# PlantandFoodResearch/MCHap

Hardware: AMD Instinct MI355X
Metric: loci/sec (whole node) for 1000-step MCMC, tetraploid 8-SNV loci, 1/2/4/8 GPUs (higher is better)
Workload: dtype f64; 1 GPU; 10000 synthetic tetraploid loci per GPU, 8 SNVs, 200 reads, 1000 MCMC steps x 2 chains, burn 500, posterior summary (BASELINE.json configs[1]); 4 passes in flight on separate HIP streams, each with its own device buffers; loci_per_gpu=10000, ploidy=4, snvs=8, reads=200, mcmc_steps=1000, chains=2, burn=500, llk_cache=True, passes_in_flight=4, hw_queues=4, world_size=1, devices=1

## Files before the change

mchap_amd/csrc/denovo_spec_kernel.hpp:

```cpp
#pragma once
#include <type_traits>

#include "denovo_simt_kernel.hpp"

#ifdef MCHAP_MASK_PADDING
#define MCHAP_PAD_LANE(x) (x)
#else
#define MCHAP_PAD_LANE(x) true
#endif
#ifndef MCHAP_COOP_UNR
#define MCHAP_COOP_UNR 2
#endif
#ifndef MCHAP_SPEC_TB
#define MCHAP_SPEC_TB 4
#endif
#ifndef MCHAP_SPEC_LOW
#define MCHAP_SPEC_LOW 8
#endif
#ifndef MCHAP_SPEC_CG
#define MCHAP_SPEC_CG 4
#endif
#ifndef MCHAP_SPEC_VAR
#define MCHAP_SPEC_VAR 0
#endif
// ... 42 lines not shown
  static __device__ __forceinline__ CT ld(u8 p) { return *reinterpret_cast<GLBP(const CT)>(p); }
};
template <>
struct TabPtr<true> {
  typedef LDSP(const uint8_t) u8;
  typedef LDSP(const double) f64;
  template <class CT>
  static __device__ __forceinline__ CT ld(u8 p) { return *reinterpret_cast<LDSP(const CT)>(p); }
};

enum { GP_RT = 0, GP_CW, GP_CT, GP_CACHE, GP_CKEYS, GP_TRACE, GP_LLK, GP_GBP, GP_N };
enum { GV_INB = 0, GV_MLO, GV_MHI, GV_N };
struct SpecLds {
  LDSP(uint64_t) pw;
  LDSP(uint64_t) wst;
  LDSP(double) llk_t;
  LDSP(uint64_t) rngn;
  LDSP(double) prior;
  LDSP(double) ptab;
  LDSP(double) optp;
  LDSP(double) optl;
  LDSP(double) ln;
  LDSP(double) lninv;
  LDSP(uint32_t) ivse;
  LDSP(uint32_t) ivlin;
  LDSP(uint32_t) ivlout;
  LDSP(uint32_t) ivno;
  LDSP(uint16_t) cols;
  LDSP(uint16_t) permtab;
  LDSP(uint8_t) shift;
  LDSP(uint8_t) nal;
  LDSP(uint8_t) ktab;
  LDSP(uint8_t) ordtab;
  LDSP(uint16_t) nreads;
  LDSP(uint16_t) ndict;
  LDSP(double) dict;
  LDSP(uint64_t) gptr;
  LDSP(double) gval;
  LDSP(uint32_t) gstream;
  LDSP(uint64_t) bw;
  LDSP(double) bpc;
  LDSP(uint64_t) bpt;
  LDSP(uint64_t) gbt;
  LDSP(const uint8_t) sct;
  LDSP(uint64_t) tbuf;
  LDSP(uint64_t) lc;
  uint32_t lc_mask;
  uint32_t cache_mask;
  int key_words;
  bool cache_on;
  uint64_t epoch = 0ull;
  bool reuse_on;
  bool cut_off = false;
  LDSP(const uint8_t) lds_ct;
  LDSP(const double) lds_cw;
  int crow;
  LDSP(uint64_t) draws;
  LDSP(double) memo_tot;
  LDSP(double) bdist;
  int memo_stride;
  int ndraws;
  LDSP(unsigned char) cx_lds;
  LDSP(double) cx_val;
  uint64_t *cx_base = nullptr;
  int cx_n = 0;
};

__host__ __device__ inline int spec_memo_entries(int Mmax) { return Mmax * (Mmax + 1) / 2; }
__host__ __device__ inline int spec_memo_index(int start, int stop) { return stop * (stop - 1) / 2 + start; }
__host__ __device__ inline size_t spec_memo_bytes(int Mmax, int T, int G) {
  const size_t per_group = (size_t)2 * spec_memo_entries(Mmax) * 8;
  if (T != 1 || per_group > 16 * 1024) return 0;
  return per_group * (64 / G);
}

constexpr int SPEC_LC_ENTRIES = 256;
#ifndef MCHAP_LC_GEN
#define MCHAP_LC_GEN 48
#endif
constexpr uint32_t SPEC_LC_SECOND_LEVEL_GEN = MCHAP_LC_GEN;
__host__ __device__ inline size_t spec_lc_bytes(int entries = SPEC_LC_ENTRIES) { return (size_t)16 * entries + 16; }
__host__ __device__ inline bool spec_ctx_in_bpc(int K, int Mmax, int Amax, int max_reads) {
  return K >= 3 && max_reads <= 64 && Mmax * Amax <= 24 * (K - 2) && 16 * K * Mmax <= 3 * 64 * 8 && 12 * 64 + 4 * 8 <= 3 * 64 * 8;
}
__host__ __device__ inline int spec_lc_entries(int bp_cache) { return (bp_cache & 2) ? ((bp_cache & 4) ? SPEC_LC_ENTRIES / 2 : SPEC_LC_ENTRIES) : 0; }
__device__ __forceinline__ uint32_t sct_off(uint32_t row) { return (row / 24u) * (uint32_t)(4 * WAVE * 8) + (row % 24u) * (uint32_t)WAVE; }
__host__ __device__ inline size_t spec_bp_cache_bytes(int K) { return (size_t)8 * K * 4 * 64 + (size_t)8 * (K + 1); }

constexpr int COAST_NW_LIST = 4;
__host__ __device__ inline size_t coast_lds_bytes(int Mmax) {
  return (size_t)8 * (2 * spec_memo_entries(Mmax) + Mmax) + (size_t)8 * 12;
}

__host__ __device__ inline size_t spec_lds_bytes(int K, int Mmax, int Amax, int T, int G) {
  const int NG = 64 / G;
  const int nmax = K * Mmax;
  const int nopt = Amax > 1 ? Amax - 1 : 1;
  const int niv = Mmax + 1;
  size_t b = 0;
  b += (size_t)8 * K * 64;
  b += (size_t)8 * NG * T * K;
  b += (size_t)8 * NG * T * 2;
  b += (size_t)8 * NG * (2 * K + 5);
  b += (size_t)8 * 64;
  b += (size_t)8 * nopt * 64 * 2;
  b += (size_t)8 * SPEC_LN * 2;
// ... 611 lines not shown
#pragma unroll
  for (int i = 0; i < RPL; i++) acc[i] = 0.0;
#pragma unroll
  for (int h = 0; h < KT; h++) {
    const uint64_t a = S.pw[(size_t)h * WAVE + src], b = S.bw[(size_t)sg * KT + h];
    const bool same = __builtin_amdgcn_readfirstlane((int)(a == b)) != 0;
    double ph[RPL];
    if (same) {
#pragma unroll
      for (int i = 0; i < RPL; i++) ph[i] = bpv[h][i];
    } else {
      spec_hap_prod<RPL, CT, LT>(dict, rows, h * Mh, Mh, ct, crow, ph);
    }
#pragma unroll
    for (int i = 0; i < RPL; i++) acc[i] += ph[i] * invK;
  }
  double wv[RPL];
#pragma unroll
  for (int i = 0; i < RPL; i++) wv[i] = cw[WAVE * i];
  return read_log_sum<RPL>(acc, wv, grouped);
}
template <int KT, int RPL, class CT, bool LT = false, class BP>
__device__ __forceinline__ void spec_base_products(const SpecLds &S, int sg, int mmax, int Mh, uint32_t amask,
                                                   typename TabPtr<LT>::u8 ct, int crow, int lane, BP &bp) {
  LDSP(double) dict = S.dict + (size_t)sg * DICT_MAX;
  const PairRows rows = spec_pair_rows<KT>(S.bw + (size_t)sg * KT, 1, 0, S, sg, mmax, Mh, amask, lane);
#pragma unroll
  for (int h = 0; h < KT; h++) {
    double ph[RPL];
    spec_hap_prod<RPL, CT, LT>(dict, rows, h * Mh, Mh, ct, crow, ph);
#pragma unroll
    for (int i = 0; i < RPL; i++) bp.set(h, i, lane, ph[i]);
  }
}
template <int KT, int RPL, class CT, bool LT = false, class BP>
__device__ __forceinline__ void spec_base_products_of(const SpecLds &S, const PairRows rows, int sg, int h, int Mh,
                                                      typename TabPtr<LT>::u8 ct, int crow, int lane, BP &bp) {
  LDSP(double) dict = S.dict + (size_t)sg * DICT_MAX;
  double ph[RPL];
  spec_hap_prod<RPL, CT, LT>(dict, rows, h * Mh, Mh, ct, crow, ph);
#pragma unroll
  for (int i = 0; i < RPL; i++) bp.set(h, i, lane, ph[i]);
}

template <int KT>
__device__ __forceinline__ unsigned long long spec_same_request(LDSP(uint64_t) pwbuf, unsigned long long reqs, int src, int lane) {
  if ((reqs & (reqs - 1ull)) == 0ull) return reqs;
  bool eq = ((reqs >> lane) & 1ull) != 0ull;
#pragma unroll
  for (int h = 0; h < KT; h++) eq = eq & (pwbuf[(size_t)h * WAVE + lane] == pwbuf[(size_t)h * WAVE + src]);
  return __ballot(eq);
}

template <int KT, int G, bool LT = false, bool DEDUP = true>
__device__ __forceinline__ double spec_coop_all(unsigned long long todo, LDSP(uint64_t) pwbuf, LDSP(uint8_t) shift_tab,
                                                LDSP(uint16_t) cols_tab, LDSP(uint16_t) nreads_tab, LDSP(uint16_t) ndict_tab,
                                                LDSP(double) dict_tab, LDSP(uint64_t) gptr_tab, LDSP(uint64_t) bw_tab,
                                                bool reuse, int crow, int mmax, int Mh_lane, uint32_t amask_lane, int rpad,
                                                int lane, LDSP(const uint8_t) lds_ct = nullptr, LDSP(const double) lds_cw = nullptr,
                                                LDSP(double) bpc = nullptr, LDSP(uint64_t) bpt = nullptr,
                                                LDSP(const uint8_t) sct = nullptr, LDSP(uint64_t) gbt = nullptr) {
  SpecLds S;
  S.pw = pwbuf;
  S.shift = shift_tab;
  S.cols = cols_tab;
  S.dict = dict_tab;
  S.bw = bw_tab;
  const int nch_batch = rpad / WAVE;
  double val = 0.0;
  while (todo) {
    const int sg = (__ffsll((long long)todo) - 1) / G;
    const unsigned long long gmask = G == 64 ? ~0ull : (((1ull << (G & 63)) - 1ull) << (sg * (G & 63)));
    unsigned long long reqs = todo & gmask;
    todo &= ~gmask;
    const int first = __ffsll((long long)reqs) - 1;
    const int Mh = __builtin_amdgcn_readfirstlane(__shfl(Mh_lane, first, WAVE));
    const uint32_t amask = (uint32_t)__builtin_amdgcn_readfirstlane(__shfl((int)amask_lane, first, WAVE));
    LDSP(uint64_t) gp = gptr_tab + sg * GP_N;
    GLBP(const double) rt = (GLBP(const double))(uintptr_t)gp[GP_RT] + lane;
    typename TabPtr<LT>::f64 cw;
    if constexpr (LT) cw = lds_cw + lane;
    else cw = (GLBP(const double))(uintptr_t)gp[GP_CW] + lane;
    const int nrd = (int)nreads_tab[sg];
    const bool grouped = nd_w01(ndict_tab[sg]);
    const int nch = max(1, min(nch_batch, (nrd + WAVE - 1) / WAVE));
    const int cstride = crow / WAVE;
    if (MCHAP_REUSE_MAXK >= KT && nd_count(ndict_tab[sg]) != 0 && KT * Mh <= (MCHAP_SPEC_DEEP ? 3 : 2) * WAVE) {
      const int nb0 = nch < 4 ? nch : 4;
      typename TabPtr<LT>::u8 ct;
      if constexpr (LT) ct = lds_ct + (size_t)lane * cstride;
      else ct = (GLBP(const uint8_t))(uintptr_t)gp[GP_CT] + (size_t)lane * cstride;
      constexpr bool BPL = (G == 64) && !LT;
      bool cached = false;
      if (BPL && bpc != nullptr) {
        bool eq = bpt[KT] != 0ull;
#pragma unroll
        for (int h = 0; h < KT; h++) eq = eq & (bpt[h] == bw_tab[(size_t)sg * KT + h]);
        cached = __builtin_amdgcn_readfirstlane((int)eq) != 0;
      }
      const bool use_base = reuse && (!BPL || bpc != nullptr) && (cached || __popcll(reqs) >= 2);
      BaseProducts<KT, BPL> bp;
      if constexpr (BPL) {
        bp.p = bpc;
      } else {
#pragma unroll
        for (int h = 0; h < KT; h++)
#pragma unroll
          for (int i = 0; i < 4; i++) bp.v[h][i] = 0.0;
      }
      if (use_base && !cached) {
        if constexpr (BPL) {
          const bool any_valid = bpt[KT] != 0ull;
#if MCHAP_SPEC_SBS
          if (sct != nullptr && nch == 1) {
// ... 293 lines not shown
                }
#pragma unroll
                for (int k = 0; k < 4; k++) acc[k] += ph[k] * invK;
              }
#pragma unroll
              for (int k = 0; k < 4; k++)
                if (k < RK) v[k] = read_log(acc[k]) * cwr[k];
            }
            const double a0 = RK > 2 ? v[0] + v[2] : v[0];
            const double a1 = RK > 3 ? v[1] + v[3] : v[1];
            double sv = RK > 1 ? a0 + a1 : a0;
#pragma unroll
            for (int o = 8; o >= 1; o >>= 1) sv += __shfl_xor(sv, o, WAVE);
#pragma unroll
            for (int k = 0; k < 4; k++) {
              const double vk = __shfl(sv, 16 * k, WAVE);
              if (k < nq && ((dupm[k] >> lane) & 1ull)) val = vk;
            }
          }
          continue;
        }
      }
#endif
      while (reqs) {
        const int src = __ffsll((long long)reqs) - 1;
        const unsigned long long dups = (DEDUP ? spec_same_request<KT>(pwbuf, reqs, src, lane) : (1ull << src));
        reqs &= ~dups;
        double s = 0.0;
        if (nb0 == 1) s += spec_coop_reuse<KT, 1, uint8_t, LT>(S, src, sg, mmax, Mh, amask, ct, cw, crow, lane, bp, use_base, grouped);
        else if (nb0 == 2) s += spec_coop_reuse<KT, 2, uint16_t, LT>(S, src, sg, mmax, Mh, amask, ct, cw, crow, lane, bp, use_base, grouped);
        else if (nb0 == 3) s += spec_coop_reuse<KT, 3, uint32_t, LT>(S, src, sg, mmax, Mh, amask, ct, cw, crow, lane, bp, use_base, grouped);
        else s += spec_coop_reuse<KT, 4, uint32_t, LT>(S, src, sg, mmax, Mh, amask, ct, cw, crow, lane, bp, use_base, grouped);
        for (int cb = 4; cb < nch; cb += 4) {
          const int rem = nch - cb;
          typename TabPtr<LT>::f64 cwb = cw + cb * WAVE;
          if (deep) {
            BaseProductsG<KT> bg;
            bg.p = gbp;
            bg.rpad = rpad;
            bg.cb = cb;
            if (rem >= 4) s += spec_coop_reuse_g<KT, 4, uint32_t, LT>(S, src, sg, mmax, Mh, amask, ct + cb, cwb, crow, lane, bg, grouped);
            else if (rem == 3) s += spec_coop_reuse_g<KT, 3, uint32_t, LT>(S, src, sg, mmax, Mh, amask, ct + cb, cwb, crow, lane, bg, grouped);
            else if (rem == 2) s += spec_coop_reuse_g<KT, 2, uint16_t, LT>(S, src, sg, mmax, Mh, amask, ct + cb, cwb, crow, lane, bg, grouped);
            else s += spec_coop_reuse_g<KT, 1, uint8_t, LT>(S, src, sg, mmax, Mh, amask, ct + cb, cwb, crow, lane, bg, grouped);
          } else {
            if (rem >= 4) s += spec_coop_coded<KT, 4, uint32_t, LT>(S, src, sg, mmax, Mh, amask, ct + cb, cwb, crow, lane, grouped);
            else if (rem == 3) s += spec_coop_coded<KT, 3, uint32_t, LT>(S, src, sg, mmax, Mh, amask, ct + cb, cwb, crow, lane, grouped);
            else if (rem == 2) s += spec_coop_coded<KT, 2, uint16_t, LT>(S, src, sg, mmax, Mh, amask, ct + cb, cwb, crow, lane, grouped);
            else s += spec_coop_coded<KT, 1, uint8_t, LT>(S, src, sg, mmax, Mh, amask, ct + cb, cwb, crow, lane, grouped);
          }
        }
        s = wave_sum(s);
        if ((dups >> lane) & 1ull) val = s;
      }
    } else {
      while (reqs) {
        const int src = __ffsll((long long)reqs) - 1;
        const unsigned long long dups = (DEDUP ? spec_same_request<KT>(pwbuf, reqs, src, lane) : (1ull << src));
        reqs &= ~dups;
        double s = 0.0;
        const bool coded = nd_count(ndict_tab[sg]) != 0;
        typename TabPtr<LT>::u8 ct;
        if constexpr (LT) ct = lds_ct + (size_t)lane * cstride;
        else ct = (GLBP(const uint8_t))(uintptr_t)gp[GP_CT] + (size_t)lane * cstride;
        GLBP(const double) cwg = (GLBP(const double))(uintptr_t)gp[GP_CW] + lane;
        for (int cb = 0; cb < nch; cb += 4) {
          const int rem = nch - cb;
          typename TabPtr<LT>::f64 cwb = cw + cb * WAVE;
          if (coded) {
            if (rem >= 4) s += spec_coop_coded<KT, 4, uint32_t, LT>(S, src, sg, mmax, Mh, amask, ct + cb, cwb, crow, lane, grouped);
            else if (rem == 3) s += spec_coop_coded<KT, 3, uint32_t, LT>(S, src, sg, mmax, Mh, amask, ct + cb, cwb, crow, lane, grouped);
            else if (rem == 2) s += spec_coop_coded<KT, 2, uint16_t, LT>(S, src, sg, mmax, Mh, amask, ct + cb, cwb, crow, lane, grouped);
            else s += spec_coop_coded<KT, 1, uint8_t, LT>(S, src, sg, mmax, Mh, amask, ct + cb, cwb, crow, lane, grouped);
          } else {
            GLBP(const double) rtb = rt + cb * WAVE;
            GLBP(const double) cwgb = cwg + cb * WAVE;
            if (rem >= 4) s += spec_coop_body<KT, 4>(S, src, sg, mmax, Mh, amask, rtb, cwgb, rpad, lane, nrd - cb * WAVE, grouped);
            else if (rem == 3) s += spec_coop_body<KT, 3>(S, src, sg, mmax, Mh, amask, rtb, cwgb, rpad, lane, nrd - cb * WAVE, grouped);
            else if (rem == 2) s += spec_coop_body<KT, 2>(S, src, sg, mmax, Mh, amask, rtb, cwgb, rpad, lane, nrd - cb * WAVE, grouped);
            else s += spec_coop_body<KT, 1>(S, src, sg, mmax, Mh, amask, rtb, cwgb, rpad, lane, nrd - cb * WAVE, grouped);
          }
        }
        s = wave_sum(s);
        if ((dups >> lane) & 1ull) val = s;
      }
    }
  }
  return val;
}

struct SpecKeepAll {
  __device__ __forceinline__ bool operator()(bool miss, double) const { return miss; }
};
template <int KT, int G, bool LT = false, class Filter = SpecKeepAll, bool DEDUP = true>
__device__ __forceinline__ double spec_eval(bool need, const GWords<KT> pw, const Grp<KT> &c, const SpecLds &S, int mmax,
                                            int rpad, int lane, Filter filt = Filter()) {
  double val = 0.0;
  if (c.flat) {
    val = c.llk;
    need = false;
  }
  bool miss = need;
  uint64_t tag = 0;
  ulonglong2 *slot = nullptr;
  GSUB_T0();
  const bool wide = C_KEYBITS(c) * KT > 63;
  uint64_t *kslot = nullptr;
  LDSP(uint64_t) lslot = S.lc;
  bool promote = false;
  if (need && S.cache_on) {
    tag = tag_of<KT>(pw, C_KEYBITS(c), S.epoch);
    const uint64_t key = tag >> 1;
    uint32_t hsh = (uint32_t)key ^ ((uint32_t)(key >> 32) * 0x9E3779B1u);
    hsh ^= hsh >> 16;
    hsh *= 0x7FEB352Du;
    hsh ^= hsh >> 15;
    hsh *= 0x846CA68Bu;
    hsh ^= hsh >> 16;
    const size_t set_i = (size_t)((hsh >> 12) & S.cache_mask);
    ulonglong2 *set = reinterpret_cast<ulonglong2 *>((uintptr_t)S.gptr[(lane / G) * GP_N + GP_CACHE]) + 8 * set_i;
    int way = (int)((hsh >> 24) & 7u);
    if (S.lc_mask != 0u && !wide) {
      LDSP(uint64_t) le = S.lc + 2 * (size_t)((hsh >> 3) & S.lc_mask);
      const uint64_t t = le[0], v = le[1];
      if (t == tag) {
        val = __longlong_as_double((long long)v);
        miss = false;
      }
      lslot = le;
      if (miss && c.gen > SPEC_LC_SECOND_LEVEL_GEN) {
#pragma unroll
        for (int w = 7; w >= 0; w--) {
          const ulonglong2 e = set[w];
          if (e.x == tag) {
            val = __longlong_as_double((long long)e.y);
            miss = false;
          }
        }
        promote = !miss;
      }
    } else {
    int hit_way = -1;
#pragma unroll
    for (int w = 7; w >= 0; w--) {
      const ulonglong2 e = set[w];
      if (e.x == tag) {
        val = __longlong_as_double((long long)e.y);
        miss = false;
        hit_way = w;
      }
      if (e.x == 0ull || (S.epoch != 0ull && (e.x ^ S.epoch) >> 33 != 0ull)) way = w;
    }
    if (wide) {
      uint64_t *kset = reinterpret_cast<uint64_t *>((uintptr_t)S.gptr[(lane / G) * GP_N + GP_CKEYS]) + 8 * set_i * S.key_words;
      if (hit_way >= 0) {
        const uint64_t *kw = kset + (size_t)hit_way * S.key_words;
        bool same = true;
#pragma unroll
        for (int h = 0; h < KT; h++) same = same & (kw[h] == pw.w[h]);
        if (!same) {
          miss = true;
          way = hit_way;
        }
      }
      kslot = kset + (size_t)way * S.key_words;
    }
    }
    slot = set + way;
  }
  if (wave_any(promote)) {
    if (promote) lslot[0] = tag;
    lds_sync();
    if (promote && lslot[0] == tag) lslot[1] = (uint64_t)__double_as_longlong(val);
    lds_sync();
  }
  miss = filt(miss, val);
  STAT_ADD(0, need);
  STAT_ADD(1, miss);
  STAT_ADD(2, true);
  unsigned long long todo = __ballot(miss);
  GSUB(c, 9);
  if (todo) {
    GCOUNT(c, 11, __popcll(todo));
    if (miss) {
#pragma unroll
      for (int h = 0; h < KT; h++) S.pw[(size_t)h * WAVE + lane] = pw.w[h];
    }
    if (S.reuse_on && lane % G == 0) {
      const GWords<KT> cg = c.g;
#pragma unroll
      for (int h = 0; h < KT; h++) S.bw[(size_t)(lane / G) * KT + h] = cg.w[h];
    }
    lds_sync();
    const double v = spec_coop_all<KT, G, LT, DEDUP>(todo, S.pw, S.shift, S.cols, S.nreads, S.ndict, S.dict, S.gptr, S.bw, S.reuse_on, S.crow, mmax, c.Mh, C_AMASK(c), rpad, lane, S.lds_ct, S.lds_cw, S.bpc, S.bpt, S.sct, S.gbt);
    if (miss) val = v;
    bool writer = miss && slot != nullptr;
    if (wave_any(writer && wide)) {
      unsigned long long pend = __ballot(writer);
      bool mine = false;
      while (pend) {
        const int l = __ffsll((long long)pend) - 1;
        const unsigned long long sl = __shfl((unsigned long long)(uintptr_t)slot, l, WAVE);
        const unsigned long long same = __ballot(writer && (unsigned long long)(uintptr_t)slot == sl);
        if (lane == l) mine = true;
        pend &= ~same;
      }
      writer = mine;
    }
    if (writer) {
      if (wide) {
#pragma unroll
        for (int h = 0; h < KT; h++) kslot[h] = pw.w[h];
      }
      *slot = make_ulonglong2(tag, (unsigned long long)__double_as_longlong(val));
    }
    if (S.lc_mask != 0u && !wide) {
      if (writer) lslot[0] = tag;
      lds_sync();
      if (writer && lslot[0] == tag) lslot[1] = (uint64_t)__double_as_longlong(val);
    }
    lds_sync();
    GSUB(c, 10);
  }
  return val;
}

#ifndef MCHAP_SPEC_WPE
#define MCHAP_SPEC_WPE 2
#endif

template <int KT, int G, bool LT = false, bool CTX = false>
__device__ __forceinline__ void spec_mutation(Grp<KT> &c, const SpecLds &S, double temp, int amax, int mmax, int nmax, int rpad,
                                              int lane, int gi, int gl) {
  const int Mh = c.Mh;
  const int n = KT * Mh;
  const uint64_t ctr0 = c.ctr;
  bool run = c.alive;
  if (wave_any(c.alive && c.mvalid)) {
    LDSP(uint64_t) utab = S.draws + gi * S.ndraws;
    const bool fast = c.alive && c.mvalid && n <= S.ndraws;
    const int cnt = max(n, min(S.ndraws, 2 * G * ((n / 2 + G) / G) - 1));
    stage_draws<G>(ld_stream(S, gi), ctr0 + (uint64_t)(n - 1), cnt, utab, gl, fast);
    lds_sync();
    bool ok = true;
    if (fast) {
      const double mlo = S.gval[gi * GV_N + GV_MLO], mhi = S.gval[gi * GV_N + GV_MHI];
      for (int p = gl; p < n; p += G) {
        const double u = draw_double(utab[p]);
        ok = ok && (mlo <= u) && (u < mhi);
      }
    }
    const bool bad = grp_ballot<G>(!ok, gi) != 0ull;
    lds_sync();
    if (fast && !bad) {
      c.ctr = ctr0 + (uint64_t)(n - 1) + (uint64_t)n;
      c.doff = n;
      c.dcount = cnt;
      run = false;
    }
  }
  if (run) c.dcount = 0;
  STAT_WAVE(8, 1);
  GPHASE(c, 0);
  if (!wave_any(run)) return;
  STAT_WAVE(9, 1);
// ... 30 lines not shown
  for (int s = 0; s < NS; s++) xs[s] = gl + s * G;
  if constexpr (G == 64) {
    const int nl = __builtin_amdgcn_readfirstlane(run ? n : 0);
    if (nl <= 64) {
      for (int i = nl - 1; i >= 1; i--) {
        const int ki = __builtin_amdgcn_readlane(kv[0], i);
        xs[0] = (xs[0] == i) ? ki : ((xs[0] == ki) ? i : xs[0]);
      }
    } else {
#pragma unroll
      for (int s2 = NS - 1; s2 >= 0; s2--) {
        const int hi = min(nl - 1, s2 * 64 + 63), lo = max(1, s2 * 64);
        for (int i = hi; i >= lo; i--) {
          const int ki = __builtin_amdgcn_readlane(kv[s2], i & 63);
#pragma unroll
          for (int s = 0; s < NS; s++) xs[s] = (xs[s] == i) ? ki : ((xs[s] == ki) ? i : xs[s]);
        }
      }
    }
  } else {
    const int nloop = run ? n : 0;
    int nl = nloop;
#pragma unroll
    for (int o = 32; o >= 1; o >>= 1) nl = max(nl, __shfl_xor(nl, o, WAVE));
    for (int i = nl - 1; i >= 1; i--) {
      if (i < nloop) {
        const int ki = ktab[i];
#pragma unroll
        for (int s = 0; s < NS; s++) xs[s] = (xs[s] == i) ? ki : ((xs[s] == ki) ? i : xs[s]);
      }
    }
  }
  if (run) {
#pragma unroll
    for (int s = 0; s < NS; s++) {
      const int e = gl + s * G;
      if (e < n) {
        int h = 0, j = e;
        while (j >= Mh) {
          j -= Mh;
          h++;
        }
        permtab[xs[s]] = (uint16_t)((h << 8) | j);
      }
    }
  }
  lds_sync();
  if (run) c.ctr = ctr0 + (uint64_t)(n - 1) + (uint64_t)n;
  const int nslots = (NS > 2 && wave_any(c.alive && n > 2 * G)) ? 3 : (two ? 2 : 1);
  const int nrd_ = (int)S.nreads[gi];
  const int wmin = (MCHAP_SPEC_SBS != 0 && G == 64 && S.bpc != nullptr && (nrd_ <= 16 || (nrd_ > 32 && nrd_ <= 64))) ? 4 : MCHAP_SPEC_WIN_MIN;
  bool cx = false;
  if constexpr (CTX && G == 64) cx = S.cx_base != nullptr && amax == 2 && run && c.gen > (uint32_t)MCHAP_CTX_GEN && c.gen >= CXP_ST(S)[CX_PAUSE];
  const bool cut_on = amax == 2 && !S.cut_off && ((S.cache_on && wave_any(c.alive && c.gen > SPEC_LC_SECOND_LEVEL_GEN)) || cx);
  int start = 0;
  int win = max(c.mwin, wmin);
  bool done = !run;
  bool any_move = false;
  double my_lo = 0.0, my_hi = 2.0;
  GT1(c, 12, t_mut0);
  while (wave_any(!done)) {
    STAT_WAVE(11, 1);
    if constexpr (CTX) STAT_WAVE(7, cx ? 1 : 0);
    bool found = false;
    int wstop = min(n, start + win);
    if constexpr (CTX && G == 64) {
      if (cx && !done) {
        ctx_acquire<KT>(c, S, n, mmax, lane);
        int fk = n, fu = n, m_h = 0;
        uint32_t m_w0 = 0, m_w1 = 0, m_l0 = 0, m_l1 = 0;
#pragma unroll 1
        for (int s = 0; s < nslots; s++) {
          const int p = gl + s * G;
          const bool in = p >= start && p < n;
          bool known = false, mv = false;
          int h = 0, sh = 0, current = 0;
          uint64_t wh = 0;
          double kllk = 0.0;
          if (in) {
            const int e = permtab[p];
            h = e >> 8;
            const int j = e & 255;
            const int ei = h * Mh + j;
            const double kpr = CXP_PR(S)[ei];
            known = kpr >= 0.0;
            if (known) {
              kllk = CXP_LLK(S, nmax)[ei];
              sh = shift[j];
              const double u = staged ? draw_double(dtab[n - 1 + p]) : stream_double(ld_stream(S, gi), ctr0 + (uint64_t)(n - 1) + (uint64_t)p);
              wh = sel_word<KT>(c.g, h);
              current = (int)((wh >> sh) & C_AMASK(c));
              const double stay = 1.0 - (0.0 + kpr);
              const double below = current == 0 ? 0.0 : 0.0 + kpr;
              my_lo = fmax(my_lo, below);
              my_hi = fmin(my_hi, below + stay);
              mv = current == 0 ? !(0.0 + stay > u) : (0.0 + kpr > u);
            }
          }
          const unsigned long long km = __ballot(known), mm = __ballot(mv), um = __ballot(in && !known);
          STAT_WAVE(5, __popcll(km));
          STAT_WAVE(6, __popcll(um));
          if (mm && fk == n) {
            const int fl = __ffsll((long long)mm) - 1;
            fk = fl + s * G;
            const uint64_t nw_ = (wh & ~((uint64_t)C_AMASK(c) << sh)) | ((uint64_t)(1 - current) << sh);
            const long long lb = __double_as_longlong(kllk);
            m_h = __builtin_amdgcn_readlane(h, fl);
            m_w0 = (uint32_t)__builtin_amdgcn_readlane((int)(uint32_t)nw_, fl);
            m_w1 = (uint32_t)__builtin_amdgcn_readlane((int)(uint32_t)(nw_ >> 32), fl);
            m_l0 = (uint32_t)__builtin_amdgcn_readlane((int)(uint32_t)lb, fl);
            m_l1 = (uint32_t)__builtin_amdgcn_readlane((int)(uint32_t)((unsigned long long)lb >> 32), fl);
          }
          if (um && fu == n) fu = __ffsll((long long)um) - 1 + s * G;
        }
        if (fk < fu || fu >= n) {
          if (fk < n) {
            set_word<KT>(c.g, m_h, (uint64_t)m_w0 | ((uint64_t)m_w1 << 32));
            c.llk = __longlong_as_double((long long)((uint64_t)m_l0 | ((uint64_t)m_l1 << 32)));
            genotype_changed<KT>(c);
            any_move = true;
            start = fk + 1;
          } else {
            start = n;
          }
          if (start >= n) done = true;
          continue;
        }
        wstop = min(fk, fu + win);
      }
    }
    const double lprior = (!done && !isnan(C_INB(S, gi))) ? prior_of<KT>(pt, C_INB(S, gi), dosage_words<KT>(c.g)) : 0.0;
#pragma unroll 1
    for (int s = 0; s < nslots; s++) {
      const int p = gl + s * G;
      bool act = !done && !found && p >= start && p < wstop;
      int h = 0, sh = 0, n_alleles = 2;
      double u = 2.0;
      if (act) {
        const int e = permtab[p];
        h = e >> 8;
        const int j = e & 255;
        if constexpr (CTX && G == 64) {
          if (cx && CXP_PR(S)[h * Mh + j] >= 0.0) act = false;
        }
        sh = shift[j];
        n_alleles = nal[j];
        u = staged ? draw_double(dtab[n - 1 + p]) : stream_double(ld_stream(S, gi), ctr0 + (uint64_t)(n - 1) + (uint64_t)p);
      }
      const uint64_t wh = sel_word<KT>(c.g, h);
      const int current = (int)((wh >> sh) & C_AMASK(c));
      const double lhapcount = S.ln[copies_of<KT>(c.g, wh)];
      const double ln_opt = S.ln[n_alleles - 1];
      double sum = 0.0;
      bool dropped = false;
#pragma unroll 1
      for (int o = 0; o < amax - 1; o++) {
        const bool prop = act && o < n_alleles - 1;
        const int i = o + (o >= current ? 1 : 0);
        GWords<KT> pw = c.g;
        const uint64_t nw = (wh & ~((uint64_t)C_AMASK(c) << sh)) | ((uint64_t)i << sh);
        set_word<KT>(pw, h, nw);
        auto known_mover_cuts = [&](bool miss, double v) -> bool {
          if (!cut_on) return miss;
          bool mv = false;
          if (prop && !miss) {
            double lprior_ratio = 0.0;
            if (!isnan(C_INB(S, gi))) lprior_ratio = prior_of<KT>(pt, C_INB(S, gi), dosage_words<KT>(pw)) - lprior;
            const double lproposal_ratio = S.ln[copies_of<KT>(pw, nw)] - lhapcount;
            const double mh = ((v - c.llk) + lprior_ratio) * temp + lproposal_ratio;
            const double pr = exp(fmin(0.0, mh) - ln_opt);
            const double stay = 1.0 - (0.0 + pr);
            mv = current == 0 ? !(0.0 + stay > u) : (0.0 + pr > u);
          }
          const uint64_t mm = grp_ballot<G>(mv, gi);
          const bool keep = miss && (mm == 0ull || gl < __ffsll((long long)mm) - 1);
          dropped = dropped || (miss && !keep);
          return keep;
        };
        GT0(t_ev);
        const double llk_i = spec_eval<KT, G, LT, decltype(known_mover_cuts), G != 64>(prop, pw, c, S, mmax, rpad, lane, known_mover_cuts);
        GT1(c, 16, t_ev);
        if (prop) {
          double lprior_ratio = 0.0;
          if (!isnan(C_INB(S, gi))) lprior_ratio = prior_of<KT>(pt, C_INB(S, gi), dosage_words<KT>(pw)) - lprior;
          const double lproposal_ratio = S.ln[copies_of<KT>(pw, nw)] - lhapcount;
          const double mh = ((llk_i - c.llk) + lprior_ratio) * temp + lproposal_ratio;
          const double pr = exp(fmin(0.0, mh) - ln_opt);
          if constexpr (CTX && G == 64) {
            if (cx && !dropped) {
              const int e_ = permtab[p];
              const int ei = (e_ >> 8) * Mh + (e_ & 255);
              CXP_PR(S)[ei] = pr;
              CXP_LLK(S, nmax)[ei] = llk_i;
              uint64_t *sp = S.cx_base + (size_t)(CXP_ST(S)[CX_CUR] - 1u) * spec_ctx_words(KT, mmax) + SPEC_CTX_HDR;
              ctx_st(sp + ei, pr);
              ctx_st(sp + nmax + ei, llk_i);
            }
          }
          S.optp[o * WAVE + lane] = pr;
          S.optl[o * WAVE + lane] = llk_i;
          sum += pr;
        }
      }
      bool changed = false;
      uint64_t neww = 0;
      double newllk = 0.0;
      if (act && !dropped) {
        const double stay = 1.0 - sum;
        double cacc = 0.0;
        int choice = -1;
        double cl = c.llk;
        for (int i = 0; i < n_alleles && choice < 0; i++) {
          double pi = stay, li = c.llk;
          if (i != current) {
            const int o = i - (i > current ? 1 : 0);
            pi = S.optp[o * WAVE + lane];
            li = S.optl[o * WAVE + lane];
          } else {
            my_lo = fmax(my_lo, cacc);
            my_hi = fmin(my_hi, cacc + stay);
          }
          cacc += pi;
          if (cacc > u) {
            choice = i;
            cl = li;
          }
        }
        if (choice < 0) {
          choice = n_alleles - 1;
          if (choice != current) cl = S.optl[(choice - (choice > current ? 1 : 0)) * WAVE + lane];
        }
        if (choice != current) {
          changed = true;
          neww = (wh & ~((uint64_t)C_AMASK(c) << sh)) | ((uint64_t)choice << sh);
          newllk = cl;
        }
      }
      const uint64_t m = grp_ballot<G>(changed, gi);
      const int fl = m ? __ffsll((long long)m) - 1 : 0;
      const int hsrc = __shfl(h, fl, G);
      const uint64_t wsrc = __shfl(neww, fl, G);
      const double lsrc = __shfl(newllk, fl, G);
      if (!done && !found && m) {
        set_word<KT>(c.g, hsrc, wsrc);
        c.llk = lsrc;
        genotype_changed<KT>(c);
        start = fl + s * G + 1;
        found = true;
      }
    }
    if (!done) {
      if (found) {
        any_move = true;
        win = max(wmin, win >> 1);
      } else {
        start = wstop;
        win = min(2 * win, 4 * G);
      }
      if (start >= n) done = true;
    }
  }
  {
    double lo = my_lo, hi = my_hi;
#pragma unroll
    for (int o = G / 2; o >= 1; o >>= 1) {
      lo = fmax(lo, __shfl_xor(lo, o, G));
      hi = fmin(hi, __shfl_xor(hi, o, G));
    }
    if (run && !any_move && c.memo_on) {
      c.mvalid = true;
      if (gl == 0) {
        S.gval[gi * GV_N + GV_MLO] = lo;
        S.gval[gi * GV_N + GV_MHI] = hi;
      }
    }
  }
  if (run) c.mwin = win;
  GPHASE(c, 1);
}

template <int KT, int G, bool PIPE = false, bool CTX = false>
__device__ __forceinline__ bool spec_structural(Grp<KT> &c, const SpecLds &S, const DenovoParams &D, int kind, double temp,
                                                const double *break_dist, int n_break_dist, int mmax, int rpad, int lane,
                                                int gi, int gl, int amax = 0) {
  const int Mh = c.Mh;
  const bool fill = PIPE && kind >= 3;
  const int step_type = (kind == 0 || kind == 3) ? 0 : 1;
  const int nivs = mmax + 1;
  LDSP(uint32_t) ivse = S.ivse + gi * nivs;
  LDSP(uint32_t) ivlin = S.ivlin + gi * nivs;
  LDSP(uint32_t) ivlout = S.ivlout + gi * nivs;
  LDSP(uint32_t) ivno = S.ivno + gi * nivs;
  LDSP(uint8_t) ord = S.ordtab + gi * nivs;
  LDSP(double) pt = S.prior + gi * (2 * KT + 5);
  bool ok = true;
  bool doit = false;
  int n_int = 0;
  LDSP(uint64_t) dtab = S.draws + gi * S.ndraws;
  if (!fill) {
    const int low = min(3 * Mh + 2, MCHAP_SPEC_LOW);
    if (wave_any(c.alive && c.dcount - c.doff < low)) {
      const int W = min(S.ndraws, 2 * G - 1);
      lds_sync();
      stage_draws<G>(ld_stream(S, gi), c.ctr, W, dtab, gl, c.alive);
      lds_sync();
      c.doff = 0;
      c.dcount = c.alive ? W : 0;
// ... 509 lines not shown
          S.cx_val = S.bpc + (size_t)((KT - 2) * 4 + 1) * WAVE;
        } else {
          p = smem + (((size_t)(p - smem) + 15) & ~(size_t)15);
          S.cx_lds = lds_cast<unsigned char>(p); p += (size_t)12 * SPEC_CTX_MAX + 4 * CX_N;
          S.cx_val = lds_cast<double>(p); p += (size_t)16 * nmax;
        }
        S.cx_n = P.ctx_n < SPEC_CTX_MAX ? P.ctx_n : SPEC_CTX_MAX;
        if (lane < CX_N) CXP_ST(S)[lane] = 0u;
        if (lane < SPEC_CTX_MAX) {
          CXP_TAG(S)[lane] = 0ull;
          CXP_STAMP(S)[lane] = 0u;
        }
      }
    }
  }
  for (int i = lane; i < SPEC_LN; i += WAVE) {
    S.ln[i] = c_ln[i];
    S.lninv[i] = c_ln_inv[i];
  }
  long long q = my_slot;
  const long long n_chains = (long long)P.n_units * Cn;
  Grp<KT> c;
  c.alive = q < n_chains;
  bool listed = false;
  if constexpr (PIPE) {
    listed = q < n_list;
    c.alive = listed;
    if (listed && P.pipe_list) q = P.pipe_list[q];
    if (!listed) q = 0;
  }
  const bool resume = PIPE && (P.pipe_mode & PIPE_RESUME);
  int base = 0;
  const int u = c.alive ? (int)(q / Cn) : 0;
  const int chain = c.alive ? (int)(q % Cn) : 0;
  const mchap_unit U = D.units[u];
  const int32_t *mi = P.meta_i + (size_t)u * meta_i_stride(P.max_pos);
  const double *mf = P.meta_f + (size_t)u * meta_f_stride(P.max_ploidy, P.max_pos, P.max_allele);
  if (c.alive && mi[META_I_STATUS] != MCHAP_UNIT_OK) c.alive = false;
  const int A = U.max_allele;
  c.Mh = c.alive ? mi[META_I_MH] : 1;
  c.bits = allele_bits(A);
  c.flat = c.alive && mi[META_I_FLAT] != 0 && !(P.flags & 128);
  if (gl == 0) {
    S.gval[gi * GV_N + GV_INB] = U.inbreeding;
    S.gval[gi * GV_N + GV_MLO] = 0.0;
    S.gval[gi * GV_N + GV_MHI] = 0.0;
    S.gstream[gi * 4 + 0] = (uint32_t)D.seed;
    S.gstream[gi * 4 + 1] = (uint32_t)(D.seed >> 32) ^ (uint32_t)(U.stream_id >> 32);
    S.gstream[gi * 4 + 2] = ((uint32_t)chain << 16) | 0u;
    S.gstream[gi * 4 + 3] = (uint32_t)U.stream_id;
  }
  S.reuse_on = !(P.flags & 8);
  S.cut_off = (P.flags & 262144) != 0;
  S.lds_ct = nullptr;
  S.lds_cw = nullptr;
  S.crow = WAVE * P.cstride;
  S.cache_on = D.cache_slots > 0 && !fillonly;
  S.cache_mask = S.cache_on ? (uint32_t)(D.cache_slots / 8) - 1u : 0u;
  S.epoch = P.cache_epoch;
  S.key_words = D.cache_key_words;
  if (gl == 0) {
    LDSP(uint64_t) gp = S.gptr + gi * GP_N;
    gp[GP_RT] = (uint64_t)(uintptr_t)(P.rt + (size_t)u * P.max_ma * rpad);
    gp[GP_CW] = (uint64_t)(uintptr_t)(P.cntw + (size_t)u * rpad);
    gp[GP_CT] = (uint64_t)(uintptr_t)(P.codes + (size_t)u * P.max_ma * WAVE * P.cstride);
    const size_t qc = (size_t)q * (size_t)(PIPE ? 1 : D.n_temps) + (size_t)tw;
    gp[GP_CACHE] = S.cache_on ? (uint64_t)(uintptr_t)(reinterpret_cast<ulonglong2 *>(D.cache) + qc * (size_t)D.cache_slots) : 0ull;
    gp[GP_CKEYS] = (S.cache_on && D.cache_keys) ? (uint64_t)(uintptr_t)(D.cache_keys + qc * (size_t)D.cache_slots * D.cache_key_words) : 0ull;
    gp[GP_TRACE] = (uint64_t)(uintptr_t)(D.trace + U.trace_off + (size_t)chain * D.steps * KT);
    gp[GP_LLK] = (uint64_t)(uintptr_t)(D.llks + U.llk_off + (size_t)chain * D.steps);
    gp[GP_GBP] = P.gbp ? (uint64_t)(uintptr_t)(P.gbp + ((size_t)q * (PIPE ? 1 : D.n_temps) + tw) * P.max_ploidy * rpad) : 0ull;
  }
  c.ctr = 0;
  c.doff = 0;
  c.dcount = 0;
  c.llk = 0.0;
  c.memo_on = (T == 1) && !(P.flags & 1);
  c.mvalid = false;
  c.mwin = MCHAP_SPEC_WIN0;
  c.fill_part = fillonly ? my_part : 0;
  c.fill_parts = fillonly ? parts_eff : 1;
  c.gen = 1;
  c.memo_gen = 1;
  if constexpr (CTX && G == 64 && PIPE) {
    if (S.cx_n > 0 && c.alive) S.cx_base = P.ctx + (size_t)q * (size_t)P.ctx_n * (size_t)spec_ctx_words(KT, mmax);
  }
  const int Mh = c.Mh;
  if (gl == 0) S.nreads[gi] = (uint16_t)(c.alive ? U.n_reads : 0);
  {
    const int nd = (c.alive && !(P.flags & 4)) ? mi[META_I_NDICT] : 0;
    if (gl == 0) S.ndict[gi] = (uint16_t)(nd | ((c.alive && mi[META_I_W01] != 0) ? (int)ND_W01 : 0));
    const double *du = P.dict + (size_t)u * DICT_MAX;
    for (int i = gl; i < nd; i += G) S.dict[(size_t)gi * DICT_MAX + i] = du[i];
  }
  S.sct = nullptr;
  if constexpr (G == 64 && MCHAP_SPEC_SBS != 0) {
    const int rows = U.n_pos * A;
    if (S.bpc != nullptr && c.alive && U.n_reads <= 64 && rows <= 24 * KT && mi[META_I_NDICT] != 0 && !(P.flags & 4)) {
      LDSP(uint8_t) t = (LDSP(uint8_t))(S.bpc + WAVE);
      GLBP(const uint8_t) ct = (GLBP(const uint8_t))(P.codes + (size_t)u * P.max_ma * WAVE * P.cstride);
      for (int r_ = 0; r_ < rows; r_++) t[sct_off((uint32_t)r_) + lane] = ct[(size_t)(r_ * WAVE + lane) * P.cstride];
      S.sct = t;
    }
  }
  if (c.alive) {
    for (int j = gl; j < Mh; j += G) {
// ... 365 lines not shown
```

mchap_amd/csrc/mchap_hip.hip:

```cpp
#include <hip/hip_runtime.h>

#include <cmath>
#include <cstdarg>
#include <cstdio>
#include <cstdlib>
#include <cstring>
#include <algorithm>
#include <atomic>
#include <mutex>
#include <vector>

#include "host_common.hpp"
#include "denovo_kernel.hpp"
#include "denovo_simt_kernel.hpp"
#include "denovo_spec_kernel.hpp"
#include "denovo_fillw_kernel.hpp"
#ifdef MCHAP_TEST_KERNELS
#include "denovo_fill_kernel.hpp"
#include "denovo_lane_kernel.hpp"
#endif

#define SPEC_LIST(X) X(2, 16) X(2, 32) X(2, 64) X(3, 16) X(3, 32) X(3, 64) X(4, 16) X(4, 32) X(4, 64) X(5, 32) X(5, 64) X(6, 32) X(6, 64) X(7, 64) X(8, 64)
#ifdef MCHAP_TEST_KERNELS
#define SPECP_LIST(X) X(2, 64) X(3, 64) X(4, 64) X(5, 64) X(6, 64) X(7, 64) X(8, 64) X(2, 16) X(3, 16) X(4, 16) X(4, 32) X(5, 32) X(6, 32)
// ... 938 lines not shown
  {
    const size_t n = (size_t)(P.max_pos + 1) * P.max_pos;
    double *bt_dev = reinterpret_cast<double *>(workspace);
    if (cfg->break_table)
      HIP_TRY(hipMemcpyAsync(bt_dev, cfg->break_table, n * sizeof(double), hipMemcpyHostToDevice, stream));
    else
      HIP_TRY(hipMemsetAsync(bt_dev, 0, n * sizeof(double), stream));
    P.break_table = bt_dev;
  }
  unsigned char *ws = reinterpret_cast<unsigned char *>(workspace) + R.bt_bytes;
  HIP_TRY(hipMemsetAsync(status, 0, sizeof(int32_t) * n_units, stream));
  P.cache = nullptr;
  P.cache_slots = 0;

  if (use_simt(cfg)) {
    const int slots = R.cache_slots;
    if (cv.ctx_n > 0) {
      SP.ctx = reinterpret_cast<uint64_t *>(ws + cv.ctx);
      SP.ctx_n = cv.ctx_n;
    }
    if (slots > 0) {
      P.cache = reinterpret_cast<uint64_t *>(ws + cv.cache);
      P.cache_slots = slots;
      uint64_t epoch = 0;
      if ((pl.kind == SAMPLER_PIPE || pl.kind == SAMPLER_SPEC) && !(T.flags & (64 | 65536)) && R.packed_bits <= 32) {
        epoch = cfg->cache_epoch > 0 ? (uint64_t)cfg->cache_epoch : g_cache_epoch.fetch_add(1) + 1;
        if (epoch >= (1ull << 31) - 1) epoch = 0;
      }
      SP.cache_epoch = epoch << 33;
      if (!epoch)
        HIP_TRY(hipMemsetAsync(ws + cv.cache, 0, R.n_caches * slots * 16, stream));
      if (cv.key_words) {
        P.cache_keys = reinterpret_cast<uint64_t *>(ws + cv.ckeys);
        P.cache_key_words = cv.key_words;
      }
    }
    SP.rt = reinterpret_cast<double *>(ws + cv.rt);
    SP.cntw = reinterpret_cast<double *>(ws + cv.cntw);
    SP.codes = ws + cv.codes;
    SP.dict = reinterpret_cast<double *>(ws + cv.dict);
    SP.gbp = (cv.has_gbp && !(T.flags & 512)) ? reinterpret_cast<double *>(ws + cv.gbp) : nullptr;
    SP.meta_i = reinterpret_cast<int32_t *>(ws + cv.meta_i);
    SP.meta_f = reinterpret_cast<double *>(ws + cv.meta_f);
    SP.lane_state = ws + cv.lane_state;
    SP.lane_memo = ws + cv.lane_memo;
    SP.pipe_state = ws + cv.pipe_state;
    SP.pipe_memo = reinterpret_cast<double *>(ws + cv.pipe_memo);
    SP.n_units = n_units;
    SP.max_pos = B.max_pos;
    SP.max_allele = B.max_allele;
    SP.max_ploidy = B.max_ploidy;
    SP.max_ma = B.max_ma;
    SP.cstride = code_stride(rpl);
    SP.flags = T.flags & (63 | 128 | 2048 | 4096 | 262144 | (1 << 20));
    SP.max_ugens_pad = (B.max_ugens + 8) & ~7;
    const size_t lds_dict = (size_t)mchap::DICT_HASH * (8 + 2) + 64;
    size_t lds_prep = (size_t)B.max_ma * rpad * 8 + (size_t)SP.max_ugens_pad * 8 + lds_dict;
    SP.prep_rows_off = 0;
    if (lds_prep > 160 * 1024 || (size_t)B.max_ma * rpad * 8 > T.prep_lds_limit) {
      lds_prep = (size_t)SP.max_ugens_pad * 8 + lds_dict;
      lds_prep = (lds_prep + 15) & ~(size_t)15;
      SP.prep_rows_off = (int)lds_prep;
      lds_prep += (size_t)B.max_allele * rpad * 8;
      SP.flags |= mchap::SIMT_FLAG_PREP_GLOBAL;
    }
    const size_t lds_simt = mchap::simt_lds_bytes(B.max_ploidy, B.max_pos, cfg->n_temps, pl.wide ? 16 : 8);
    SP.word_bits = pl.wide ? 128 : 64;
    if (lds_prep > 160 * 1024 || lds_simt > 160 * 1024)
      return fail(MCHAP_ERR_LIMIT, "a unit needs %zu / %zu bytes of LDS (> 160 KiB)", lds_prep, lds_simt);
    auto prepare = [&](const mchap::SimtParams &Q, int n, hipStream_t st) {
      switch (rpl) {
        case 1: return launch_prepare<1>(Q, n, lds_prep, st);
        case 2: return launch_prepare<2>(Q, n, lds_prep, st);
        case 3: return launch_prepare<3>(Q, n, lds_prep, st);
        case 4: return launch_prepare<4>(Q, n, lds_prep, st);
        case 5: return launch_prepare<5>(Q, n, lds_prep, st);
        case 6: return launch_prepare<6>(Q, n, lds_prep, st);
        case 7: return launch_prepare<7>(Q, n, lds_prep, st);
        case 8: return launch_prepare<8>(Q, n, lds_prep, st);
        case 12: return launch_prepare<12>(Q, n, lds_prep, st);
        case 16: return launch_prepare<16>(Q, n, lds_prep, st);
        case 24: return launch_prepare<24>(Q, n, lds_prep, st);
        case 32: return launch_prepare<32>(Q, n, lds_prep, st);
        case 48: return launch_prepare<48>(Q, n, lds_prep, st);
        default: return launch_prepare<64>(Q, n, lds_prep, st);
      }
    };
    rc = prepare(SP, n_units, stream);
    if (rc) return rc;
    switch (pl.kind) {
#ifdef MCHAP_TEST_KERNELS
      case SAMPLER_LANE: return launch_lane(T, pl.K, SP, n_units, cfg->chains, cfg->timer, stream);
#endif
      case SAMPLER_PIPE:
        return launch_pipe(T, pl.K, pl.G, SP, n_units, cfg->chains, reinterpret_cast<int32_t *>(ws + cv.pipe_lists),
                           reinterpret_cast<int32_t *>(ws + cv.pipe_counts), cfg->timer, stream, B.min_reads <= 64, B.max_reads, R.packed_bits);
      case SAMPLER_SPEC: return launch_spec(T, pl.K, pl.G, SP, n_units, cfg->chains, cfg->n_temps, cfg->timer, stream);
      default: return launch_simt(pl.K, SP, n_units, cfg->chains, lds_simt, cfg->timer, stream, pl.wide);
    }
  }

#ifdef MCHAP_TEST_KERNELS
  size_t lds = 0;
  for (int u = 0; u < n_units; u++) {
    const mchap_unit &U = units_host[u];
    const mchap::WaveLayout L = mchap::wave_layout(U.ploidy, U.n_pos, U.max_allele, cfg->n_temps);
    const int cpb = cfg->chains < mchap::CHAINS_PER_BLOCK ? cfg->chains : mchap::CHAINS_PER_BLOCK;
// ... 186 lines not shown
```

Before: 1.179 million loci/s.

## Stop cooperative likelihood evaluation early once any proposal in window accepts

Adds a stop predicate to the cooperative spec evaluation loop so that, once a served likelihood yields an accepted Metropolis move for any lane, the remaining requested evaluations in the wave are abandoned. Unserved lanes are marked as dropped, and the cache write is rekeyed from the shared LDS proposal words. By default (stop_mode 1) the scan window is pinned at its maximum width instead of adaptively shrinking. The aim is to skip likelihood evaluations past the first mover, at the cost of extra ballots, rehashing, and wider windows that may waste work when moves are rare.

```diff
diff --git a/mchap_amd/csrc/denovo_spec_kernel.hpp b/mchap_amd/csrc/denovo_spec_kernel.hpp
--- a/mchap_amd/csrc/denovo_spec_kernel.hpp
+++ b/mchap_amd/csrc/denovo_spec_kernel.hpp
@@ -118,6 +118,7 @@
   uint64_t epoch = 0ull;
   bool reuse_on;
   bool cut_off = false;
+  int stop_mode = 0;
   LDSP(const uint8_t) lds_ct;
   LDSP(const double) lds_cw;
   int crow;
@@ -835,14 +836,23 @@
   return __ballot(eq);
 }
 
-template <int KT, int G, bool LT = false, bool DEDUP = true>
+struct SpecNeverStop {
+  __device__ __forceinline__ bool operator()(unsigned long long, unsigned long long, double) const { return false; }
+};
+template <bool ON, class F>
+__device__ __forceinline__ auto spec_stop_if(F f) {
+  if constexpr (ON) return f;
+  else return SpecNeverStop();
+}
+template <int KT, int G, bool LT = false, bool DEDUP = true, class Stop = SpecNeverStop>
 __device__ __forceinline__ double spec_coop_all(unsigned long long todo, LDSP(uint64_t) pwbuf, LDSP(uint8_t) shift_tab,
                                                 LDSP(uint16_t) cols_tab, LDSP(uint16_t) nreads_tab, LDSP(uint16_t) ndict_tab,
                                                 LDSP(double) dict_tab, LDSP(uint64_t) gptr_tab, LDSP(uint64_t) bw_tab,
                                                 bool reuse, int crow, int mmax, int Mh_lane, uint32_t amask_lane, int rpad,
                                                 int lane, LDSP(const uint8_t) lds_ct = nullptr, LDSP(const double) lds_cw = nullptr,
                                                 LDSP(double) bpc = nullptr, LDSP(uint64_t) bpt = nullptr,
-                                                LDSP(const uint8_t) sct = nullptr, LDSP(uint64_t) gbt = nullptr) {
+                                                LDSP(const uint8_t) sct = nullptr, LDSP(uint64_t) gbt = nullptr,
+                                                Stop stop = Stop(), unsigned long long *left = nullptr) {
   SpecLds S;
   S.pw = pwbuf;
   S.shift = shift_tab;
@@ -1242,6 +1252,11 @@
         }
         s = wave_sum(s);
         if ((dups >> lane) & 1ull) val = s;
+        if (stop(dups, reqs | todo, val)) {
+          if (left != nullptr) *left = reqs | todo;
+          reqs = 0ull;
+          todo = 0ull;
+        }
       }
     } else {
       while (reqs) {
@@ -1273,18 +1288,41 @@
         }
         s = wave_sum(s);
         if ((dups >> lane) & 1ull) val = s;
+        if (stop(dups, reqs | todo, val)) {
+          if (left != nullptr) *left = reqs | todo;
+          reqs = 0ull;
+          todo = 0ull;
+        }
       }
     }
   }
   return val;
 }
 
+__device__ __forceinline__ uint32_t spec_key_hash(uint64_t key) {
+  uint32_t hsh = (uint32_t)key ^ ((uint32_t)(key >> 32) * 0x9E3779B1u);
+  hsh ^= hsh >> 16;
+  hsh *= 0x7FEB352Du;
+  hsh ^= hsh >> 15;
+  hsh *= 0x846CA68Bu;
+  hsh ^= hsh >> 16;
+  return hsh;
+}
+template <class T>
+struct SpecStops {
+  static constexpr bool value = true;
+};
+template <>
+struct SpecStops<SpecNeverStop> {
+  static constexpr bool value = false;
+};
 struct SpecKeepAll {
   __device__ __forceinline__ bool operator()(bool miss, double) const { return miss; }
 };
-template <int KT, int G, bool LT = false, class Filter = SpecKeepAll, bool DEDUP = true>
+template <int KT, int G, bool LT = false, class Filter = SpecKeepAll, bool DEDUP = true, class Stop = SpecNeverStop>
 __device__ __forceinline__ double spec_eval(bool need, const GWords<KT> pw, const Grp<KT> &c, const SpecLds &S, int mmax,
-                                            int rpad, int lane, Filter filt = Filter()) {
+                                            int rpad, int lane, Filter filt = Filter(), Stop stop = Stop(),
+                                            bool *unserved = nullptr) {
   double val = 0.0;
   if (c.flat) {
     val = c.llk;
@@ -1298,18 +1336,13 @@
   uint64_t *kslot = nullptr;
   LDSP(uint64_t) lslot = S.lc;
   bool promote = false;
+  int way = 0;
   if (need && S.cache_on) {
     tag = tag_of<KT>(pw, C_KEYBITS(c), S.epoch);
-    const uint64_t key = tag >> 1;
-    uint32_t hsh = (uint32_t)key ^ ((uint32_t)(key >> 32) * 0x9E3779B1u);
-    hsh ^= hsh >> 16;
-    hsh *= 0x7FEB352Du;
-    hsh ^= hsh >> 15;
-    hsh *= 0x846CA68Bu;
-    hsh ^= hsh >> 16;
+    const uint32_t hsh = spec_key_hash(tag >> 1);
     const size_t set_i = (size_t)((hsh >> 12) & S.cache_mask);
     ulonglong2 *set = reinterpret_cast<ulonglong2 *>((uintptr_t)S.gptr[(lane / G) * GP_N + GP_CACHE]) + 8 * set_i;
-    int way = (int)((hsh >> 24) & 7u);
+    way = (int)((hsh >> 24) & 7u);
     if (S.lc_mask != 0u && !wide) {
       LDSP(uint64_t) le = S.lc + 2 * (size_t)((hsh >> 3) & S.lc_mask);
       const uint64_t t = le[0], v = le[1];
@@ -1366,12 +1399,10 @@
   }
   miss = filt(miss, val);
   STAT_ADD(0, need);
-  STAT_ADD(1, miss);
   STAT_ADD(2, true);
   unsigned long long todo = __ballot(miss);
   GSUB(c, 9);
   if (todo) {
-    GCOUNT(c, 11, __popcll(todo));
     if (miss) {
 #pragma unroll
       for (int h = 0; h < KT; h++) S.pw[(size_t)h * WAVE + lane] = pw.w[h];
@@ -1382,9 +1413,27 @@
       for (int h = 0; h < KT; h++) S.bw[(size_t)(lane / G) * KT + h] = cg.w[h];
     }
     lds_sync();
-    const double v = spec_coop_all<KT, G, LT, DEDUP>(todo, S.pw, S.shift, S.cols, S.nreads, S.ndict, S.dict, S.gptr, S.bw, S.reuse_on, S.crow, mmax, c.Mh, C_AMASK(c), rpad, lane, S.lds_ct, S.lds_cw, S.bpc, S.bpt, S.sct, S.gbt);
-    if (miss) val = v;
-    bool writer = miss && slot != nullptr;
+    unsigned long long left = 0ull;
+    const double v = spec_coop_all<KT, G, LT, DEDUP, Stop>(todo, S.pw, S.shift, S.cols, S.nreads, S.ndict, S.dict, S.gptr, S.bw, S.reuse_on, S.crow, mmax, c.Mh, C_AMASK(c), rpad, lane, S.lds_ct, S.lds_cw, S.bpc, S.bpt, S.sct, S.gbt, stop, &left);
+    const bool served = miss && ((left >> lane) & 1ull) == 0ull;
+    GCOUNT(c, 11, __popcll(todo & ~left));
+    STAT_ADD(1, served);
+    if (served) val = v;
+    if (unserved != nullptr) *unserved = miss && !served;
+    GWords<KT> kw = pw;
+    if constexpr (SpecStops<Stop>::value) {
+      const bool again = miss && S.cache_on;
+#pragma unroll
+      for (int h = 0; h < KT; h++) kw.w[h] = S.pw[(size_t)h * WAVE + lane];
+      tag = tag_of<KT>(kw, C_KEYBITS(c), S.epoch);
+      const uint32_t hsh = spec_key_hash(tag >> 1);
+      const size_t set_i = (size_t)((hsh >> 12) & S.cache_mask);
+      ulonglong2 *set = reinterpret_cast<ulonglong2 *>((uintptr_t)S.gptr[(lane / G) * GP_N + GP_CACHE]) + 8 * set_i;
+      slot = again ? set + way : nullptr;
+      lslot = S.lc + 2 * (size_t)((hsh >> 3) & S.lc_mask);
+      kslot = reinterpret_cast<uint64_t *>((uintptr_t)S.gptr[(lane / G) * GP_N + GP_CKEYS]) + (8 * set_i + (size_t)way) * S.key_words;
+    }
+    bool writer = served && slot != nullptr;
     if (wave_any(writer && wide)) {
       unsigned long long pend = __ballot(writer);
       bool mine = false;
@@ -1400,7 +1449,7 @@
     if (writer) {
       if (wide) {
 #pragma unroll
-        for (int h = 0; h < KT; h++) kslot[h] = pw.w[h];
+        for (int h = 0; h < KT; h++) kslot[h] = kw.w[h];
       }
       *slot = make_ulonglong2(tag, (unsigned long long)__double_as_longlong(val));
     }
@@ -1537,9 +1586,12 @@
   const int wmin = (MCHAP_SPEC_SBS != 0 && G == 64 && S.bpc != nullptr && (nrd_ <= 16 || (nrd_ > 32 && nrd_ <= 64))) ? 4 : MCHAP_SPEC_WIN_MIN;
   bool cx = false;
   if constexpr (CTX && G == 64) cx = S.cx_base != nullptr && amax == 2 && run && c.gen > (uint32_t)MCHAP_CTX_GEN && c.gen >= CXP_ST(S)[CX_PAUSE];
-  const bool cut_on = amax == 2 && !S.cut_off && ((S.cache_on && wave_any(c.alive && c.gen > SPEC_LC_SECOND_LEVEL_GEN)) || cx);
+  constexpr bool STOP = (G == 64) && !LT;
+  const bool stop_on = STOP && S.stop_mode != 0 && amax == 2 && !S.cut_off && !(MCHAP_SPEC_SBS != 0 && nrd_ <= 64);
+  const bool fullwin = stop_on && S.stop_mode == 1;
+  const bool cut_on = amax == 2 && !S.cut_off && (stop_on || (S.cache_on && wave_any(c.alive && c.gen > SPEC_LC_SECOND_LEVEL_GEN)) || cx);
   int start = 0;
-  int win = max(c.mwin, wmin);
+  int win = fullwin ? 4 * G : max(c.mwin, wmin);
   bool done = !run;
   bool any_move = false;
   double my_lo = 0.0, my_hi = 2.0;
@@ -1645,30 +1697,38 @@
         GWords<KT> pw = c.g;
         const uint64_t nw = (wh & ~((uint64_t)C_AMASK(c) << sh)) | ((uint64_t)i << sh);
         set_word<KT>(pw, h, nw);
+        double lprior_ratio = 0.0, lproposal_ratio = 0.0;
+        if (prop) {
+          if (!isnan(C_INB(S, gi))) lprior_ratio = prior_of<KT>(pt, C_INB(S, gi), dosage_words<KT>(pw)) - lprior;
+          lproposal_ratio = S.ln[copies_of<KT>(pw, nw)] - lhapcount;
+        }
+        auto moves = [&](double v) -> bool {
+          const double mh = ((v - c.llk) + lprior_ratio) * temp + lproposal_ratio;
+          const double pr = exp(fmin(0.0, mh) - ln_opt);
+          const double stay = 1.0 - (0.0 + pr);
+          return current == 0 ? !(0.0 + stay > u) : (0.0 + pr > u);
+        };
         auto known_mover_cuts = [&](bool miss, double v) -> bool {
           if (!cut_on) return miss;
           bool mv = false;
-          if (prop && !miss) {
-            double lprior_ratio = 0.0;
-            if (!isnan(C_INB(S, gi))) lprior_ratio = prior_of<KT>(pt, C_INB(S, gi), dosage_words<KT>(pw)) - lprior;
-            const double lproposal_ratio = S.ln[copies_of<KT>(pw, nw)] - lhapcount;
-            const double mh = ((v - c.llk) + lprior_ratio) * temp + lproposal_ratio;
-            const double pr = exp(fmin(0.0, mh) - ln_opt);
-            const double stay = 1.0 - (0.0 + pr);
-            mv = current == 0 ? !(0.0 + stay > u) : (0.0 + pr > u);
-          }
+          if (prop && !miss) mv = moves(v);
           const uint64_t mm = grp_ballot<G>(mv, gi);
           const bool keep = miss && (mm == 0ull || gl < __ffsll((long long)mm) - 1);
           dropped = dropped || (miss && !keep);
           return keep;
         };
+        auto stop_at_mover = [&](unsigned long long served, unsigned long long, double v) -> bool {
+          if (!stop_on) return false;
+          bool mv = false;
+          if ((served >> lane) & 1ull) mv = moves(v);
+          return __ballot(mv) != 0ull;
+        };
+        bool unserved = false;
         GT0(t_ev);
-        const double llk_i = spec_eval<KT, G, LT, decltype(known_mover_cuts), G != 64>(prop, pw, c, S, mmax, rpad, lane, known_mover_cuts);
+        const double llk_i = spec_eval<KT, G, LT, decltype(known_mover_cuts), G != 64>(prop, pw, c, S, mmax, rpad, lane, known_mover_cuts, spec_stop_if<STOP>(stop_at_mover), &unserved);
         GT1(c, 16, t_ev);
+        dropped = dropped || unserved;
         if (prop) {
-          double lprior_ratio = 0.0;
-          if (!isnan(C_INB(S, gi))) lprior_ratio = prior_of<KT>(pt, C_INB(S, gi), dosage_words<KT>(pw)) - lprior;
-          const double lproposal_ratio = S.ln[copies_of<KT>(pw, nw)] - lhapcount;
           const double mh = ((llk_i - c.llk) + lprior_ratio) * temp + lproposal_ratio;
           const double pr = exp(fmin(0.0, mh) - ln_opt);
           if constexpr (CTX && G == 64) {
@@ -1737,7 +1797,7 @@
     if (!done) {
       if (found) {
         any_move = true;
-        win = max(wmin, win >> 1);
+        if (!fullwin) win = max(wmin, win >> 1);
       } else {
         start = wstop;
         win = min(2 * win, 4 * G);
@@ -2353,6 +2413,7 @@
   }
   S.reuse_on = !(P.flags & 8);
   S.cut_off = (P.flags & 262144) != 0;
+  S.stop_mode = (G != 64 || (P.flags & 2097152)) ? 0 : ((P.flags & 4194304) ? 2 : 1);
   S.lds_ct = nullptr;
   S.lds_cw = nullptr;
   S.crow = WAVE * P.cstride;
diff --git a/mchap_amd/csrc/mchap_hip.hip b/mchap_amd/csrc/mchap_hip.hip
--- a/mchap_amd/csrc/mchap_hip.hip
+++ b/mchap_amd/csrc/mchap_hip.hip
@@ -1014,7 +1014,7 @@
     SP.max_ploidy = B.max_ploidy;
     SP.max_ma = B.max_ma;
     SP.cstride = code_stride(rpl);
-    SP.flags = T.flags & (63 | 128 | 2048 | 4096 | 262144 | (1 << 20));
+    SP.flags = T.flags & (63 | 128 | 2048 | 4096 | 262144 | (1 << 20) | (1 << 21) | (1 << 22));
     SP.max_ugens_pad = (B.max_ugens + 8) & ~7;
     const size_t lds_dict = (size_t)mchap::DICT_HASH * (8 + 2) + 64;
     size_t lds_prep = (size_t)B.max_ma * rpad * 8 + (size_t)SP.max_ugens_pad * 8 + lds_dict;
```

After: 1.167 million loci/s. 0.99x the previous value.
